# dariopagliaricci/Metal-PathTracer-arm64

Measured on AMD Instinct MI355X. Metric: Msamples/sec (whole node) at 1920×1080, depth 8; PFM RMSE vs Embree ref, higher is better.
Workload: dtype f32; 1 GPU; BASELINE configs[1]: Cornell box + one 70,688-triangle OBJ mesh, 1920x1080, depth 8, 256 spp, seed 1337; partition=8-row bands round-robin over 1 rank(s), RCCL gather of the HDR buffer

## Files before the change

### metal-pathtracer-arm64_amd/csrc/host/device_scene.h

```cpp
#pragma once

#include <hip/hip_runtime.h>

#include <cstdio>
#include <cstring>
#include <exception>
#include <functional>
#include <memory>
#include <string>
#include <vector>

#include "../kernels/device_types.h"
#include "../kernels/launch.h"
#include "env_importance_sampler.h"
#include "geometry_cache.h"
#include "ptr_abi.h"

namespace ptrhost {

struct HipError {
    std::string message;
};

#define HIP_CHECK(expr)                                                                                     \
// ... 88 lines not shown

}

struct PtrDeviceScene {
    int device = 0;
    DeviceBuffer<uint4> qnodes;
    DeviceBuffer<uint4> wnodes;
    DeviceBuffer<float4> nodes, tris, triNormals, spheres, materials, rects, rectLights, envRgba;
    DeviceBuffer<uint2> sphereInfo;
    DeviceBuffer<int32_t> lightIndexByRect;
    DeviceBuffer<float2> envCond, envMarg, cone;
    DeviceBuffer<float4> triUv, triTangent, texels, materialTex;
    DeviceBuffer<uint4> texInfo;
    DeviceBuffer<float> envPdf;
    DeviceBuffer<float4> envMips;
    uint32_t envMipLevels = 0;
    ptrk::SceneView view{};
    std::unique_ptr<ptrhost::DynamicScene> dynamic;
    uint64_t info[8] = {0};
    double uploadSeconds = 0.0;
    double timings[4] = {0.0, 0.0, 0.0, 0.0};
    uint64_t deviceTotalBytes = 0;
    bool hasRandomWalkMaterial = false;

    DeviceBuffer<float4> state, recBuf, itemAccum;
    DeviceBuffer<float2> hit;
    DeviceBuffer<uint32_t> flushItem, signature, tailList, tailWords;
    DeviceBuffer<uint32_t> connectList, connectCounts;
    DeviceBuffer<uint32_t> busyLists, busyCounts;
    uint64_t tailBelow = 512ull << 10;
    uint64_t poolSlots = 32ull << 20;
    uint32_t poolGroups = 0;
    bool connectOverlap = true;
    uint32_t maxPoolGroups() const { return poolGroups ? poolGroups : 4u; }
    uint32_t feederChunk = 256;
    std::vector<hipStream_t> groupStreams;
    std::vector<hipEvent_t> groupEvents;
    std::vector<hipStream_t> sideStreams;
    std::vector<hipEvent_t> sideEvents;
    int refillBelow = 40;
    uint32_t spillLevels = 0;
    uint32_t wideDepth = 0;
    DeviceBuffer<uint4> medium;
    DeviceBuffer<float> envLod;
    DeviceBuffer<uint32_t> scalars, pixelOfLocal, spill;
    DeviceBuffer<uint2> itemReserve;
    DeviceBuffer<uint32_t> itemHeads, zeros;
    DeviceBuffer<uint64_t> counters;
    DeviceBuffer<float> outBands;
    DeviceBuffer<float> covBands;
    DeviceBuffer<float4> covMean;
    ptrhost::AdaptiveStore adaptive;
    DeviceBuffer<float> adaptiveOut;
    DeviceBuffer<float4> rayBatch;
    DeviceBuffer<PtrHit> hitBatch;
    uint32_t* pinnedAlive = nullptr;
    uint32_t traceGrid = 0;
    uint32_t traceGridHalf = 0;
    uint32_t cachedW = 0, cachedH = 0, cachedPart = 0, cachedParts = 0, cachedLocalPixels = 0;

    ~PtrDeviceScene() {
        if (pinnedAlive) (void)hipHostFree(pinnedAlive);
        for (hipStream_t st : groupStreams) (void)hipStreamDestroy(st);
        for (hipEvent_t e : groupEvents) (void)hipEventDestroy(e);
        for (hipStream_t st : sideStreams) (void)hipStreamDestroy(st);
        for (hipEvent_t e : sideEvents) (void)hipEventDestroy(e);
// ... 73 lines not shown
```

### metal-pathtracer-arm64_amd/csrc/host/hip_backend.cpp

```cpp
#include <hip/hip_runtime.h>

#include <algorithm>
#include <chrono>
#include <cmath>
#include <cstdio>
#include <cstdlib>
#include <cstring>
#include <exception>
#include <memory>
#include <string>
#include <functional>
#include <vector>

#include "bvh_builder.h"
#include "device_scene.h"
#include "env_importance_sampler.h"
#include "geometry_cache.h"
#include "knobs.h"
#include "ptr_dynamic.h"
#include "scene_geometry.h"
#include "vecmath.h"

using namespace ptrk;
using namespace ptrhost;
// ... 257 lines not shown
        ds.texels.upload(reinterpret_cast<const float4*>(ps.texels.data()), ps.texels.size() / 4);
        ds.texInfo.upload(reinterpret_cast<const uint4*>(ps.texInfo.data()), ps.texInfo.size() / 4);
        ds.materialTex.upload(reinterpret_cast<const float4*>(ps.materialTex.data()), ps.materialTex.size() / 4);
        v.triUv = ds.triUv.ptr;
        v.triTangent = ds.triTangent.ptr;
        v.texels = ds.texels.ptr;
        v.texInfo = ds.texInfo.ptr;
        v.materialTex = ds.materialTex.ptr;
        v.textureCount = desc.textureCount;
    }

    if (ps.dynamic) uploadDynamicTables(ps, ds);

    ds.info[0] = bvh.nodeCount;
    ds.info[1] = bvh.leafCount;
    ds.info[2] = triCount;
    ds.info[3] = desc.sphereCount;
    ds.info[4] = bvh.maxDepth;
    ds.info[5] = bvh.maxLeafSize;
    ds.info[6] = static_cast<uint64_t>(bvh.sahCost * 1000.0);
    ds.info[7] = lightCount;

    hipDeviceProp_t prop;
    HIP_CHECK(hipGetDeviceProperties(&prop, ds.device));
    ds.deviceTotalBytes = prop.totalGlobalMem;
    const uint32_t cus = prop.multiProcessorCount > 0 ? static_cast<uint32_t>(prop.multiProcessorCount) : 256u;
    ds.traceGrid = cus * 8u;
    if (knobs.refillBelow > 0) ds.refillBelow = knobs.refillBelow;
    ds.traceGridHalf = cus * 4u;
    if (knobs.tailBelow >= 0) ds.tailBelow = static_cast<uint64_t>(knobs.tailBelow);
    if (knobs.poolSlots != 0) ds.poolSlots = knobs.poolSlots;
    if (knobs.poolGroups != 0) ds.poolGroups = knobs.poolGroups;
    ds.connectOverlap = knobs.connectOverlap != 0;
    const uint32_t wideLevels = ps.pg.wideCount > 0u ? ps.pg.wideDepth : 0u;
    const uint32_t stackNeed = std::min<uint32_t>(kTraversalStackDepth, std::max(3u * wideLevels, static_cast<uint32_t>(bvh.maxDepth)) + 4u);
    v.stackLimit = std::max(stackNeed, kLdsStackLevels);
    ds.wideDepth = wideLevels;
    ds.spillLevels = v.stackLimit - kLdsStackLevels;
    ds.spill.ensure(std::max<size_t>(spillWordsPerGroup(ds) * ds.maxPoolGroups() * 2u, 1u));
    ds.scalars.ensure(static_cast<size_t>(kScalarCount) * kMaxPoolGroups);
    ds.counters.ensure(kCounterSlots);
    ds.zeros.ensure(16);
    HIP_CHECK(hipMemset(ds.zeros.ptr, 0, 16 * sizeof(uint32_t)));
    HIP_CHECK(hipHostMalloc(reinterpret_cast<void**>(&ds.pinnedAlive), sizeof(uint32_t) * (kPinnedHeadsOffset + kItemHeads), hipHostMallocDefault));
    const double copySeconds = std::chrono::duration<double>(std::chrono::steady_clock::now() - t0).count();
    ds.uploadSeconds = ps.seconds + copySeconds;
    ds.timings[0] = ps.geometrySeconds;
    ds.timings[1] = ps.shadingSeconds;
    ds.timings[2] = copySeconds;
    ds.timings[3] = ps.geometryFromCache ? 1.0 : 0.0;
    if (knobs.verboseBuild) std::fprintf(stderr, "[upload] prepare %.2f s, copies to the device %.2f s\n", ps.seconds, copySeconds);
}

}

namespace {

int uploadTo(const char* who, const PtrSceneDesc* scene, const char* cachePath, int device, PtrDeviceScene** outScene, char* err, size_t cap,
             bool dynamic = false) {
    if (!scene || !outScene) return nullArgument(who, err, cap);
    if (ptr_device_count() <= device || device < 0) {
        setErr(err, cap, std::string(who) + ": no such HIP device (the HIP path has no CPU fallback)");
        return 2;
    }
    try {
        auto ds = std::make_unique<PtrDeviceScene>();
// ... 80 lines not shown
    rp.byWidth = makeDivU32(s.width);
    rp.height = s.height;
    rp.maxDepth = std::min(s.maxDepth, kFlagFieldMask);
    rp.shadowSlack = (s.debugShadowSlack > 0.0f && s.debugShadowSlack < 1.0f) ? s.debugShadowSlack : 0.0f;
    rp.seedBase = s.seed != 0 ? s.seed : 0x9e3779b9u;
    rp.spp = std::max(1u, spp);
    rp.sampleBase = 0u;
    rp.sppTotal = rp.spp;
    rp.passFlags = 3u;
    rp.enableRussianRoulette = s.enableRussianRoulette;
    rp.enableSpecularNee = s.enableSpecularNee;
    rp.enableMnee = s.enableMnee;
    rp.enableMneeSecondary = s.enableMneeSecondary;
    rp.backgroundMode = s.backgroundMode;
    std::memcpy(rp.backgroundColor, s.backgroundColor, sizeof(rp.backgroundColor));
    rp.envRotation = s.environmentRotation;
    rp.envIntensity = s.environmentIntensity;
    rp.clampFactor = std::max(s.fireflyClampFactor, 0.0f);
    rp.clampFloor = std::max(s.fireflyClampFloor, 0.0f);
    rp.throughputClamp = std::max(s.throughputClamp, 0.0f);
    rp.tailClampBase = std::max(s.specularTailClampBase, 0.0f);
    rp.tailClampRoughnessScale = std::max(s.specularTailClampRoughnessScale, 0.0f);
    rp.minSpecularPdf = std::max(s.minSpecularPdf, 1.0e-8f);
    rp.clampEnabled = s.fireflyClampEnabled ? 1.0f : 0.0f;
    rp.emissionScale = (s.emissionScale > 0.0f && std::isfinite(s.emissionScale)) ? s.emissionScale : 1.0f;
    rp.mediaMode = s.metalSemantics & (PTR_METAL_MEDIA | PTR_METAL_THIN | PTR_METAL_FACE_NORMAL | PTR_METAL_SPECULAR | PTR_METAL_SSS | PTR_METAL_PBR |
                                       PTR_METAL_CLAMPS | PTR_METAL_ENV_LOD | PTR_METAL_RAY_DIFF);
    rp.clampMaxContribution = std::max(s.fireflyClampMaxContribution, 0.0f);
    rp.minSpecularPdfRaw = s.minSpecularPdf;
    rp.sssMode = s.sssMode;
    rp.sssMaxSteps = std::max(s.sssMaxSteps, 1u);
}

LaunchConfig coldLaunchConfig(const PtrDeviceScene& ds) { return LaunchConfig{ds.traceGrid, ds.spill.ptr, ds.scalars.ptr + 1, ds.refillBelow}; }

void partitionPixels(uint32_t width, uint32_t height, uint32_t part, uint32_t parts, std::vector<uint32_t>& out) {
    out.clear();
    const uint32_t bands = (height + PTR_BAND_ROWS - 1u) / PTR_BAND_ROWS;
    for (uint32_t b = part; b < bands; b += parts) {
        const uint32_t y0 = b * PTR_BAND_ROWS, y1 = std::min(y0 + PTR_BAND_ROWS, height);
        for (uint32_t ty = y0; ty < y1; ty += 8u) {
            for (uint32_t tx = 0; tx < width; tx += 8u) {
                for (uint32_t y = ty; y < std::min(ty + 8u, y1); ++y) {
                    for (uint32_t x = tx; x < std::min(tx + 8u, width); ++x) out.push_back(y * width + x);
                }
            }
        }
    }
}

void addLaunchStats(PtrRenderStats& a, const PtrRenderStats& b) {
    a.traceKernelMs += b.traceKernelMs;
    a.shadeKernelMs += b.shadeKernelMs;
    a.shadowKernelMs += b.shadowKernelMs;
    a.tailKernelMs += b.tailKernelMs;
    a.traceLaunches += b.traceLaunches;
    a.samples += b.samples;
}

}

namespace {

uint64_t itemBudgetBytes(const PtrDeviceScene& ds) {
    return std::max<uint64_t>(64ull << 20, std::min<uint64_t>(16ull << 30, ds.deviceTotalBytes / 4u));
}

// ... 110 lines not shown
        ds.sideEvents.push_back(newEvent());
    }
}

std::vector<PoolGroup> makeGroups(PtrDeviceScene& ds, const RenderParams& rp, bool count, bool soloGroup, uint32_t slots, hipStream_t stream) {
    const uint32_t wantGroups = ds.poolGroups ? ds.poolGroups : (slots > (8u << 20) ? 2u : 4u);
    uint32_t groupCount = std::min<uint32_t>(soloGroup ? 1u : wantGroups, std::max<uint32_t>(1u, slots >> 20));
    const uint32_t groupSlots = ((slots + groupCount - 1u) / groupCount + 255u) & ~255u;
    groupCount = (slots + groupSlots - 1u) / groupSlots;
    const bool overlap = ds.connectOverlap && !soloGroup && groupCount <= 2u;
    ensureGroupStreams(ds, groupCount, overlap);
    const size_t spillWords = spillWordsPerGroup(ds);
    const uint32_t connectRegion = ((groupSlots + 63u) / 64u + kConnectQueues - 1u) / kConnectQueues * 64u;
    const size_t connectListWords = static_cast<size_t>(connectRegion) * kConnectQueues;
    if (slots >= (1u << kConnectMaskShift)) throw HipError{"path-slot pool too large for the connect lists"};
    ds.connectList.ensure(connectListWords * groupCount);
    ds.connectCounts.ensure(kConnectCountWords * 2u * kMaxPoolGroups);
    ds.busyLists.ensure(connectListWords * 2u * groupCount);
    ds.busyCounts.ensure(kConnectCountWords * 3u * kMaxPoolGroups);
    std::vector<PoolGroup> groups(groupCount);
    for (uint32_t g = 0; g < groupCount; ++g) {
        PoolGroup& gr = groups[g];
        const uint32_t first = g * groupSlots;
        gr.pool = slotRange(ds, rp, count, slots, first, std::min(groupSlots, slots - first), gr.env);
        gr.pool.connectList = ds.connectList.ptr + connectListWords * g;
        gr.pool.connectRegion = connectRegion;
        gr.listWords = connectListWords;
        gr.connectCounts = ds.connectCounts.ptr + kConnectCountWords * 2u * g;
        gr.busyLists = ds.busyLists.ptr + connectListWords * 2u * g;
        gr.busyCounts = ds.busyCounts.ptr + kConnectCountWords * 3u * g;
        gr.scalars = ds.scalars.ptr + static_cast<size_t>(g) * kScalarCount;
        const bool sideBySide = groupCount > 1 && gr.pool.slots >= kHalfGridGroupSlots;
        gr.cfg = LaunchConfig{sideBySide ? ds.traceGridHalf : ds.traceGrid, ds.spill.ptr + g * spillWords, gr.scalars + 1, ds.refillBelow};
        gr.stream = g == 0 ? stream : ds.groupStreams[g - 1];
        gr.feederChunk = ds.feederChunk;
        if (overlap) {
            gr.side = ds.sideStreams[g];
            gr.shadeDone = ds.sideEvents[2 * g];
            gr.connectDone = ds.sideEvents[2 * g + 1];
            gr.sideSpill = ds.spill.ptr + (ds.maxPoolGroups() + g) * spillWords;
        }
    }
    return groups;
}

uint64_t itemRangeStart(const RenderParams& rp, uint32_t k) {
    return std::min<uint64_t>(static_cast<uint64_t>(rp.itemHeadFirst) + static_cast<uint64_t>(k) * rp.itemsPerHead, rp.itemCount);
}

constexpr uint64_t kPollEvery = 4;
constexpr uint64_t kPollDry = 2;

struct PollResult {
    bool allDone, runTail, queueDry;
    uint64_t nextCheck;
};

PollResult poll(PtrDeviceScene& ds, std::vector<PoolGroup>& groups, const RenderParams& rp, uint32_t slots, uint64_t iterations, bool queueDry,
                bool tracePolls) {
    HIP_CHECK(hipGetLastError());
    const uint32_t ring = static_cast<uint32_t>((iterations - 1u) % kAliveRing);
    bool headsCopied = false;
    for (uint32_t g = 0; g < groups.size(); ++g) {
        PoolGroup& gr = groups[g];
        if (gr.done) continue;
        if (queueDry) {
// ... 527 lines not shown
```

### metal-pathtracer-arm64_amd/csrc/host/knobs.cpp

```cpp
#include "knobs.h"

#include <algorithm>
#include <cstdlib>
#include <cstring>

namespace ptr {

namespace {

long long numberOr(const char* name, long long fallback) {
    const char* e = std::getenv(name);
    if (!e || !*e) return fallback;
    char* end = nullptr;
    const long long v = std::strtoll(e, &end, 10);
    return end == e ? fallback : v;
}

bool hasTopic(const char* list, const char* topic) {
    if (!list) return false;
    const size_t n = std::strlen(topic);
    for (const char* p = list; *p;) {
        const char* q = std::strchr(p, ',');
        const size_t len = q ? static_cast<size_t>(q - p) : std::strlen(p);
        if ((len == n && std::strncmp(p, topic, n) == 0) || (len == 3 && std::strncmp(p, "all", 3) == 0)) return true;
        p += len + (q ? 1 : 0);
    }
    return false;
}

}

Knobs readKnobs() {
    Knobs k;
    k.poolSlots = static_cast<uint64_t>(std::min<long long>(std::max<long long>(numberOr("PTR_POOL_SLOTS", 0), 0), 64ll << 20));
    if (k.poolSlots != 0 && k.poolSlots < 1024) k.poolSlots = 1024;
    k.poolGroups = static_cast<uint32_t>(std::min<long long>(std::max<long long>(numberOr("PTR_POOL_GROUPS", 0), 0), 8));
    k.connectOverlap = static_cast<int>(numberOr("PTR_CONNECT_OVERLAP", -1));
    k.wideNodes = static_cast<int>(numberOr("PTR_WIDE_NODES", -1));
    k.quantizedNodes = static_cast<int>(numberOr("PTR_QUANTIZED_NODES", -1));
    k.tailBelow = numberOr("PTR_TAIL_BELOW", -1);
    k.maxItems = static_cast<uint64_t>(std::max<long long>(numberOr("PTR_MAX_ITEMS", 0), 0));
    if (k.maxItems != 0 && k.maxItems < 1024) k.maxItems = 1024;
    k.refillBelow = static_cast<int>(std::min<long long>(std::max<long long>(numberOr("PTR_REFILL_BELOW", 0), 0), 64));
    k.buildThreads = static_cast<uint32_t>(std::min<long long>(std::max<long long>(numberOr("PTR_BUILD_THREADS", 0), 0), 256));
    k.noOversize = numberOr("PTR_NO_OVERSIZE", 0) != 0;
    k.denoiseTiled = static_cast<int>(numberOr("PTR_DENOISE_TILED", -1));
    const char* verbose = std::getenv("PTR_VERBOSE");
    k.verboseBuild = hasTopic(verbose, "build");
    k.verbosePolls = hasTopic(verbose, "polls");
    k.verboseLaunches = hasTopic(verbose, "launches");
    k.verboseSteps = hasTopic(verbose, "steps");
    return k;
}

}
```

### metal-pathtracer-arm64_amd/csrc/host/knobs.h

```cpp
#pragma once

#include <cstdint>

namespace ptr {

struct Knobs {
    uint64_t poolSlots = 0;
    uint32_t poolGroups = 0;
    int connectOverlap = -1;
    int wideNodes = -1;
    int quantizedNodes = -1;
    int64_t tailBelow = -1;
    uint64_t maxItems = 0;
    int refillBelow = 0;
    uint32_t buildThreads = 0;
    bool noOversize = false;
    int denoiseTiled = -1;
    bool verboseBuild = false, verbosePolls = false, verboseLaunches = false, verboseSteps = false;
};

Knobs readKnobs();

}
```

### metal-pathtracer-arm64_amd/csrc/kernels/device_types.h

```cpp
#pragma once

#include <cstdint>
#include <hip/hip_runtime.h>

#include "bvh_layout.h"

namespace ptrk {

struct SceneView {
    const float4* nodes;
    const uint4* qnodes;
    float gridOrigin[3];
    float gridCell[3];
    float gridInvCell[3];
    uint32_t useQuantized;
    const float4* tris;
    const float4* triNormals;
    const float4* spheres;
    const uint2* sphereInfo;
    const float4* materials;
    const float4* rects;
    const float4* rectLights;
    const int32_t* lightIndexByRect;
    const float4* envRgba;
// ... 92 lines not shown
    uint32_t sssMode;
    uint32_t sssMaxSteps;
    uint32_t itemHeadFirst;
    uint32_t itemsPerHead;
    uint32_t enableRussianRoulette, enableSpecularNee, enableMnee, enableMneeSecondary;
    uint32_t backgroundMode;
    float backgroundColor[3];
    float envRotation, envIntensity;
    float clampFactor, clampFloor, throughputClamp, tailClampBase, tailClampRoughnessScale, minSpecularPdf, clampEnabled;
    float emissionScale;
    float clampMaxContribution, minSpecularPdfRaw;
    float shadowSlack;
};

struct EnvLodView {
    const float4* mips;
    float* slotLod;
    uint32_t levels;
    uint32_t pad;
};

struct ShadowRecordView {
    float4* org;
    float4* dir;
    float4* a;
    float4* b;
};

constexpr uint32_t kItemHeads = 64u;
constexpr uint32_t kItemHeadStride = 64u;
constexpr uint32_t kItemHeadWords = kItemHeads * kItemHeadStride + 1u;

constexpr uint32_t kRecSlots = 5u;

struct PathPool {
    float4* ray0;
    float4* ray1;
    float2* hit;
    float4* thr;
    float4* accum;
    uint32_t* flushItem;
    uint4* medium;
    float2* cone;
    uint32_t* signature;
    float4* itemAccum;
    uint32_t* nextItem;
    ShadowRecordView rec[kRecSlots];
    uint2* itemReserve;
    const uint32_t* pixelOfLocal;
    const float4* zero;
    uint64_t* counters;
    uint32_t slots;
    uint32_t recStride;
    uint32_t* connectList;
    uint32_t* connectCount;
    uint32_t* connectClear;
    uint32_t connectRegion;
    const uint32_t* busyIn;
    const uint32_t* busyCountIn;
    uint32_t* busyOut;
    uint32_t* busyCountOut;
    uint32_t* busyCountClear;
};
constexpr uint32_t kBusyAliveBit = 1u << 31;
constexpr uint32_t kConnectQueues = 64u;
constexpr uint32_t kConnectCountStride = 64u;
// ... 74 lines not shown
```

### metal-pathtracer-arm64_amd/csrc/kernels/launch.h

```cpp
#pragma once

#include <hip/hip_runtime.h>

#include "device_types.h"
#include "ptr_abi.h"

namespace ptrk {

struct LaunchConfig {
    uint32_t traceGrid;
    uint32_t* spill;
    uint32_t* workCounters;
    int refillBelow;
    uint32_t feederChunk = 256;
};

void launchGenerate(const RenderParams& rp, const PathPool& pool, hipStream_t stream);
int traversalNodeFormat(const SceneView& sc, bool count);
void launchExtend(const SceneView& sc, const PathPool& pool, const LaunchConfig& cfg, uint32_t* aliveOut, bool count, hipStream_t stream);
struct ShadeResets {
    uint32_t* extendHead;
    uint32_t* connectHead;
    uint32_t* nextAlive;
    uint32_t drained;
};
void launchShade(const RenderParams& rp, const SceneView& sc, const PathPool& pool, const ShadeResets& resets, const EnvLodView& env, bool count,
                 hipStream_t stream);
uint32_t shadeKernelSet(const RenderParams& rp, const SceneView& sc, bool count);
void launchConnect(const RenderParams& rp, const SceneView& sc, const PathPool& pool, const LaunchConfig& cfg, bool count,
                   hipStream_t stream);
void launchTail(const RenderParams& rp, const SceneView& sc, const PathPool& pool, const EnvLodView& env, const LaunchConfig& cfg, uint32_t* dList,
                uint32_t* dListCount, uint32_t* dListHead, bool count, hipStream_t stream);
void launchResolve(const RenderParams& rp, const PathPool& pool, uint32_t partCount, float* dOut, hipStream_t stream);
void launchResolveCov(const RenderParams& rp, const PathPool& pool, uint32_t partCount, float4* dMean, float* dCov, hipStream_t stream);

void launchTraceRays(const SceneView& sc, const float4* dRays, uint64_t n, bool anyHit, PtrHit* dOut, const LaunchConfig& cfg,
                     uint64_t* dCounters, hipStream_t stream);

void launchAovs(const RenderParams& rp, const SceneView& sc, uint32_t sample, float4* dAlbedo, float4* dNormal, const LaunchConfig& cfg,
                hipStream_t stream);

void launchDebugEvalBsdf(const float4* dMaterial, const RenderParams& rp, const float* dIn, uint64_t n, float* dOut,
                         hipStream_t stream);
void launchDebugSampleBsdf(const float4* dMaterial, const RenderParams& rp, const float* dIn, const uint32_t* dFront,
                           const uint32_t* dRng, uint64_t n, float* dOut, uint32_t* dRngOut, hipStream_t stream);
void launchDebugSampleLobes(const float4* dMaterial, const RenderParams& rp, const float* dIn, const uint32_t* dFront, const uint32_t* dRng,
                            uint64_t n, float* dOut, float* dSample, uint32_t* dRngOut, hipStream_t stream);
// ... 20 lines not shown
```

### metal-pathtracer-arm64_amd/csrc/kernels/wavefront.hip

```cpp
#include <hip/hip_runtime.h>

#include <algorithm>

#include "bsdf.h"
#include "device_types.h"
#include "launch.h"
#include <type_traits>
#include "traverse.h"
#include "texture.h"
#include "vec.h"

namespace ptrk {

namespace {

constexpr float kEps = 1.0e-4f;
constexpr float kSpecNeePdfFloor = 1.0e-4f;
constexpr float kSpecNeeInvPdfClamp = 1.0e4f;
constexpr float kMisMin = 1.0e-4f;
constexpr float kMisMax = 0.9999f;
#ifndef PTR_SHADE_BLOCK
#define PTR_SHADE_BLOCK 128
#endif
constexpr uint32_t kShadeBlock = PTR_SHADE_BLOCK;
// ... 1422 lines not shown
                        const bool dirValid = finite3(bs.dir);
                        const bool mneeEligible = rp.enableMnee && bs.isDelta && dirValid && type == 2u && nextSpecDepth == 1u;
                        const bool specNeeEligible = rp.enableSpecularNee && bs.isDelta && dirValid && !mneeEligible;

                        if (specNeeEligible || mneeEligible) {
                            const f3 sdir = normalize(bs.dir);
                            const f3 sorg = offsetOrigin(of, sdir);
                            if (envSampling) {
                                const SpecularLightWeight w = specularLightWeight(envPdfOf(sc, sdir, rp.envRotation), bs.pdf);
                                const f3 envColor = envLookup(sc, sdir, rp.envRotation, rp.envIntensity);
                                const f3 contrib = (bs.weight * envColor) * (w.mis * w.invPdf);
                                if (finite3(contrib)) {
                                    const f3 clamped = clampFirefly(thr, contrib, cc);
                                    if (clamped.x > 0.0f || clamped.y > 0.0f || clamped.z > 0.0f) {
                                        storeRecord(pool, slot, 2u, 0u, sorg, INFINITY, sdir, clamped, 0.0f, mk3(0.0f));
                                        want[2] = true;
                                    }
                                }
                            }
                            if (sc.rectLightCount > 0u && sc.settleRectLights) {
                                if (COUNT) counts.settled += 1u;
                                float tl;
                                uint32_t li = 0u, half = 0u;
                                if (nearestRectLight(sc, sorg, sdir, tl, li, half)) {
                                    uint32_t ignore;
                                    const Surface ls = rectLightSurface(sc, sorg, sdir, tl, li, half, ignore);
                                    const f3 c = rectContributionAt(rp, sc, cc, ls, sorg, bs.weight, bs.pdf, thr);
                                    if (c.x != 0.0f || c.y != 0.0f || c.z != 0.0f) {
                                        storeRecord(pool, slot, 3u, 3u, sorg, tl, sdir, c, 0.0f, mk3(__uint_as_float(ignore), 0.0f, 0.0f));
                                        want[3] = true;
                                    }
                                }
                            } else if (sc.rectLightCount > 0u) {
                                storeRecord(pool, slot, 3u, 1u, sorg, INFINITY, sdir, bs.weight, bs.pdf, thr);
                                want[3] = true;
                            }
                        }
                        if (mneeEligible && rp.enableMneeSecondary) {
                            const f3 sdir = normalize(bs.dir);
                            storeRecord(pool, slot, 4u, 2u, offsetOrigin(of, sdir), __uint_as_float(rng), sdir, bs.weight, bs.pdf, thr);
                            want[4] = true;
                        }

                        thr *= bs.weight;
                        thr = clampThroughput(thr, cc);
                        const float maxComp = smax(smax(thr.x, thr.y), thr.z);
                        if (!finite3(thr) || maxComp <= 0.0f) {
                            endPath = true;
                        } else {
                            lastPdf = bs.pdf > 0.0f ? bs.pdf : lastPdf;
                            lastDelta = bs.isDelta;
                            if (envLodOn && bs.lobe == 1 && !bs.isDelta && env.levels > 1u) {
                                envLodNext = envLodFromRoughness(bs.lobeRoughness, static_cast<float>(env.levels - 1u));
                            }
                            nextO = (SSS && bs.hasExit) ? sssExitOrigin(bs.exitPoint, n, bs.dir) : offsetOrigin(of, bs.dir);
                            nextD = bs.dir;
                            if (TEX && pool.cone) {
                                if (!haveCone) cone = pool.cone[slot];
                                haveCone = true;
                                cone.x = smax(cone.x + cone.y * smax(hitv.x, 0.0f), 1.0e-7f);
                                float inc = 0.0f;
                                if (!bs.isDelta) {
                                    const bool pbr = cc.metalPbr && type == 7u;
                                    const int lobe = pbr ? bs.lobe : ((type == 0u || type == 5u) ? 0 : 1);
                                    const float r = clampf(pbr ? bs.lobeRoughness : mat.roughness01(), 0.0f, 1.0f);
                                    inc = lobe == 0 ? 0.55f : (lobe == 1 ? 0.03f + (0.45f - 0.03f) * r : 0.10f + (0.60f - 0.10f) * r);
                                }
// ... 202 lines not shown
    f3 result = mk3(0.0f);
    if (COUNT) ++raysClosest;
    const TraceHit h = traverse<false, COUNT>(sc, org, dir, kEps, INFINITY, stack, cntClosest);
    if (h.prim == kHitMiss || sc.materialCount == 0u) return result;
    const Surface cs = reconstruct(sc, org, dir, h.t, h.prim);
    f3 tmpE;
    float tmpP;
    if (sc.rectLightCount > 0u && rectLightHit(sc, cs, org, rp.emissionScale, tmpE, tmpP)) return result;
    const Mat cm{sc.materials + static_cast<size_t>(min(cs.material, sc.materialCount - 1u)) * kMaterialVec4};
    if (!materialIsDelta(cm)) return result;
    f3 cn = cs.normal;
    if (dot(cn, cn) <= 0.0f) cn = mk3(0.0f, 1.0f, 0.0f);
    cn = normalize(cn);
    const f3 cin = normalize(dir);
    const BsdfSampleResult s2 = sampleBsdf(cm, cs.position, cn, -cin, cin, cs.frontFace, rngCopy, cc);
    if (!(s2.pdf > 0.0f && s2.isDelta && dot(s2.dir, s2.dir) > 0.0f && finite3(s2.weight))) return result;
    const f3 d2 = normalize(s2.dir);
    const f3 o2 = offsetOrigin(cs, d2);
    const f3 w2 = weight * s2.weight;
    const float pdf2 = bsdfPdf * s2.pdf;
    if (sc.envSampling) {
        if (COUNT) ++raysAny;
        result += alongEnv<COUNT>(rp, sc, cc, o2, d2, w2, pdf2, thr, stack, cntAny);
    }
    if (sc.rectLightCount > 0u) {
        if (COUNT) ++raysClosest;
        result += alongRect<COUNT>(rp, sc, cc, o2, d2, w2, pdf2, thr, stack, cntClosest);
    }
    return result;
}

}

template <bool COUNT, int NODES>
__global__ void __launch_bounds__(kTraceBlock) PTR_EXTEND_ATTR k_connect(RenderParams rp, SceneView sc, PathPool pool, uint32_t* spill, uint32_t spillStride,
                                                          uint32_t* workCounter, int kRefillBelow, uint32_t feederChunk) {
    __shared__ uint32_t ldsStack[kLdsStackLevels * kTraceBlock];
    LaneStack stack = laneStack(ldsStack, spill, spillStride, sc);
    TraceCounters cnt{0u, 0u}, cntClosest{0u, 0u};
    uint32_t rays = 0u, raysClosest = 0u, early = 0u;
    const ClampCfg cc = clampCfg(rp);

    SceneMem mem = sceneMem(sc);
    SubLists lists;
    lists.init(pool.connectCount, pool.connectRegion);
    WaveFeeder feeder;
    feeder.init(workCounter, lists.total, shortListChunk(lists.total, (gridDim.x * blockDim.x) >> 6));
    Trav t;
    t.cur = 0u;
    bool active = false;
    uint32_t mySlot = 0u, bits = 0u;
    float4* const recBase = pool.rec[0].org;
    const uint32_t slots = pool.recStride;
    uint32_t myRecAt = 0u;
    while (true) {
        const int nActive = __popcll(__ballot(active));
        const bool idleBits = __ballot(!active && bits != 0u) != 0ull;
        if (nActive < kRefillBelow && (idleBits || !feeder.exhausted)) {
            if (!feeder.exhausted) {
                const uint32_t idx = feeder.take(!active && bits == 0u);
                const uint32_t at = lists.position(idx != WaveFeeder::kNone ? idx : 0u, pool.connectRegion);
                if (idx != WaveFeeder::kNone) {
                    const uint32_t entry = pool.connectList[at];
                    mySlot = entry & ((1u << kConnectMaskShift) - 1u);
                    bits = entry >> kConnectMaskShift;
                }
            }
            if (!active && bits != 0u) {
                const uint32_t rec = static_cast<uint32_t>(__ffs(static_cast<int>(bits))) - 1u;
                bits &= bits - 1u;
                myRecAt = rec * 4u * slots + mySlot;
                const float4 o4 = recBase[myRecAt], d4 = recBase[myRecAt + slots];
                const uint32_t kind = __float_as_uint(d4.w);
                if (kind != 2u) {
                    const bool any = kind != 1u;
                    if (COUNT) { if (any) ++rays; else ++raysClosest; }
                    active = travBegin<NODES>(sc, t, mk3(o4), mk3(d4), kEps, any ? o4.w : INFINITY, any, stack);
                    if (kind == 3u) t.hit.prim = __float_as_uint(recBase[myRecAt + 3u * slots].x);
                    if (!active && kind == 1u) recBase[myRecAt + 2u * slots] = make_float4(0.0f, 0.0f, 0.0f, 0.0f);
                }
            }
            continue;
        }
        if (nActive == 0) break;
        {
            TraceCounters step{0u, 0u};
            const bool more = travVote<COUNT, NODES>(sc, mem, t, active, stack, step);
            if (COUNT) {
                TraceCounters& dst = t.anyHit ? cnt : cntClosest;
                dst.nodes += step.nodes;
                dst.prims += step.prims;
            }
            if (!more) {
                active = false;
                float4* const a = recBase + myRecAt + 2u * slots;
                if (t.anyHit) {
                    if (COUNT) early += anyHitFound(t.hit.prim) ? 1u : 0u;
                    if (anyHitFound(t.hit.prim)) *a = make_float4(0.0f, 0.0f, 0.0f, 0.0f);
                } else {
                    const float4 a4 = *a;
                    const f3 c = rectContribution(rp, sc, cc, t.org, t.dir, t.hit, mk3(a4), a4.w, mk3(recBase[myRecAt + 3u * slots]));
                    *a = mk4(c, 0.0f);
                }
            }
        }
    }
    addTraceCounters<COUNT>(pool.counters, rays, cnt, raysClosest, cntClosest);
    if (COUNT) addCounter(pool.counters, kCntShadowEarlyExit, early);
}

template <bool COUNT>
__global__ void __launch_bounds__(kTraceBlock) k_connect_chain(RenderParams rp, SceneView sc, PathPool pool, uint32_t* spill, uint32_t spillStride) {
    __shared__ uint32_t ldsStack[kLdsStackLevels * kTraceBlock];
    const uint32_t gtid = blockIdx.x * kTraceBlock + threadIdx.x;
    LaneStack stack = laneStack(ldsStack, spill, spillStride, sc);
    TraceCounters cnt{0u, 0u}, cntClosest{0u, 0u};
    uint32_t rays = 0u, raysClosest = 0u;
    const ClampCfg cc = clampCfg(rp);
    for (uint32_t slot = gtid; slot < pool.slots; slot += gridDim.x * kTraceBlock) {
        if (!((__float_as_uint(pool.ray1[slot].w) >> kFlagPendingShift) & (1u << 4))) continue;
        const ShadowRecordView& r = pool.rec[4];
        const float4 d4 = r.dir[slot];
        if (__float_as_uint(d4.w) != 2u) continue;
        const float4 o4 = r.org[slot], a4 = r.a[slot];
        const f3 c = mneeChain<COUNT>(rp, sc, cc, mk3(o4), mk3(d4), __float_as_uint(o4.w), mk3(a4), a4.w, mk3(r.b[slot]), stack, cnt,
                                      cntClosest, rays, raysClosest);
        r.a[slot] = mk4(c, 0.0f);
    }
    addTraceCounters<COUNT>(pool.counters, rays, cnt, raysClosest, cntClosest);
}

__global__ void __launch_bounds__(256) k_tail_collect(PathPool pool, uint32_t* list, uint32_t* listCount) {
    __shared__ uint32_t found[4][64];
    const uint32_t wave = threadIdx.x >> 6, lane = laneId();
    const uint32_t wavesTotal = gridDim.x * 4u;
    const uint32_t waveId = blockIdx.x * 4u + wave;
    const uint32_t perWave = ((pool.slots + wavesTotal - 1u) / wavesTotal + 63u) & ~63u;
    const uint32_t begin = waveId * perWave, end = min(begin + perWave, pool.slots);
    uint32_t have = 0u;
    auto flush = [&]() {
        uint32_t base = 0u;
// ... 554 lines not shown
    const uint32_t needs = sc.materialTypes | ((sc.envWidth > 0u || sc.envSampling) ? kFeatureEnvironment : 0u) |
                           ((rp.mediaMode & (PTR_METAL_MEDIA | PTR_METAL_FACE_NORMAL)) ? kFeatureMedia : 0u);
    for (uint32_t set : {kDiffuseMaterials, kBasicMaterials, kMetalMaterials, kCarPaintMaterials, kPbrMaterials}) {
        if ((needs & ~set) == 0u) {
            v.set = set;
            break;
        }
    }
    return v;
}

uint32_t shadeKernelSet(const RenderParams& rp, const SceneView& sc, bool count) { return shadeVariant(rp, sc, count).set; }

void launchShade(const RenderParams& rp, const SceneView& sc, const PathPool& pool, const ShadeResets& resets, const EnvLodView& env, bool count,
                 hipStream_t stream) {
    const ShadeVariant v = shadeVariant(rp, sc, count);
    const bool listed = pool.busyIn != nullptr;
    const uint32_t grid = ceilDiv(pool.slots, kShadeBlock);
    auto launch = [&](auto kernel) { hipLaunchKernelGGL(kernel, dim3(grid), dim3(kShadeBlock), 0, stream, rp, sc, pool, resets, env); };
    withBools([&](auto countTag, auto listedTag) {
        constexpr bool C = decltype(countTag)::value, L = decltype(listedTag)::value;
        if (v.tex) launch(k_shade<C, true, true, L>);
        else if (v.sss) launch(k_shade<C, true, false, L>);
        else if (C) launch(k_shade<C, false, false, L>);
        else if (v.set == kDiffuseMaterials) launch(k_shade<false, false, false, L, kDiffuseMaterials>);
        else if (v.set == kBasicMaterials) launch(k_shade<false, false, false, L, kBasicMaterials>);
        else if (v.set == kMetalMaterials) launch(k_shade<false, false, false, L, kMetalMaterials>);
        else if (v.set == kCarPaintMaterials) launch(k_shade<false, false, false, L, kCarPaintMaterials>);
        else if (v.set == kPbrMaterials) launch(k_shade<false, false, false, L, kPbrMaterials>);
        else launch(k_shade<C, false, false, L>);
    }, count, listed);
}

void launchConnect(const RenderParams& rp, const SceneView& sc, const PathPool& pool, const LaunchConfig& cfgIn, bool count, hipStream_t stream) {
    const TraceLaunch t = traceLaunch(cfgIn);
    withNodeFormat(sc, count, [&](auto countTag, auto nodesTag) {
        hipLaunchKernelGGL((k_connect<decltype(countTag)::value, decltype(nodesTag)::value>), dim3(t.grid), dim3(kTraceBlock), 0, stream, rp, sc, pool,
                           t.cfg.spill, t.stride, t.cfg.workCounters + 1, t.cfg.refillBelow, t.cfg.feederChunk);
    });
    if (rp.enableMnee && rp.enableMneeSecondary) {
        withBools([&](auto countTag) {
            hipLaunchKernelGGL(k_connect_chain<decltype(countTag)::value>, dim3(t.grid), dim3(kTraceBlock), 0, stream, rp, sc, pool, t.cfg.spill, t.stride);
        }, count);
    }
}

void launchTail(const RenderParams& rp, const SceneView& sc, const PathPool& pool, const EnvLodView& env, const LaunchConfig& cfgIn, uint32_t* dList,
                uint32_t* dListCount, uint32_t* dListHead, bool count, hipStream_t stream) {
    const TraceLaunch t = traceLaunch(cfgIn);
    const uint32_t collectGrid = std::max(1u, std::min(t.grid, ceilDiv(pool.slots, 256u * 16u)));
    hipLaunchKernelGGL(k_tail_collect, dim3(collectGrid), dim3(256), 0, stream, pool, dList, dListCount);
    const ShadeVariant v = shadeVariant(rp, sc, count);
    withBools([&](auto countTag, auto sssTag, auto texTag) {
        constexpr bool C = decltype(countTag)::value, S = decltype(sssTag)::value, T = decltype(texTag)::value;
        hipLaunchKernelGGL((k_tail_run<C, S, S && T>), dim3(t.grid), dim3(kTraceBlock), 0, stream, rp, sc, pool, dList, dListCount, dListHead,
                           t.cfg.spill, t.stride, env);
    }, count, v.sss, v.tex);
}

void launchResolve(const RenderParams& rp, const PathPool& pool, uint32_t partCount, float* dOut, hipStream_t stream) {
    hipLaunchKernelGGL(k_flush, dim3(ceilDiv(pool.slots, 256)), dim3(256), 0, stream, rp, pool);
    hipLaunchKernelGGL(k_resolve, dim3(ceilDiv(rp.localPixels, 256)), dim3(256), 0, stream, rp, pool, partCount, dOut);
}

void launchTraceRays(const SceneView& sc, const float4* dRays, uint64_t n, bool anyHit, PtrHit* dOut, const LaunchConfig& cfgIn,
                     uint64_t* dCounters, hipStream_t stream) {
    const TraceLaunch t = traceLaunch(cfgIn, n);
    withBools([&](auto anyTag) {
        hipLaunchKernelGGL(k_trace_rays<decltype(anyTag)::value>, dim3(t.grid), dim3(kTraceBlock), 0, stream, sc, dRays, n, dOut, t.cfg.spill, t.stride,
                           dCounters);
    }, anyHit);
}
// ... 78 lines not shown
```

Measured before the change: 2526 Msamples/s.

## Split rect-light contribution out of connect traversal into a settle kernel

The connect kernel no longer takes RenderParams or evaluates rect-light contributions inline. It is templated on whether closest-hit records are traced, and for closest hits it only stores the hit distance and primitive. A new k_connect_settle kernel then computes rectContribution for those records. This is meant to slim the traversal kernel (fewer registers, simpler code, and a variant that skips closest records entirely when they are not needed), at the cost of an extra launch and an extra round trip through memory for the records.

```diff
diff --git a/metal-pathtracer-arm64_amd/csrc/host/device_scene.h b/metal-pathtracer-arm64_amd/csrc/host/device_scene.h
--- a/metal-pathtracer-arm64_amd/csrc/host/device_scene.h
+++ b/metal-pathtracer-arm64_amd/csrc/host/device_scene.h
@@ -144,6 +144,7 @@
     uint64_t poolSlots = 32ull << 20;
     uint32_t poolGroups = 0;
     bool connectOverlap = true;
+    bool connectAllKinds = false;
     uint32_t maxPoolGroups() const { return poolGroups ? poolGroups : 4u; }
     uint32_t feederChunk = 256;
     std::vector<hipStream_t> groupStreams;
diff --git a/metal-pathtracer-arm64_amd/csrc/host/hip_backend.cpp b/metal-pathtracer-arm64_amd/csrc/host/hip_backend.cpp
--- a/metal-pathtracer-arm64_amd/csrc/host/hip_backend.cpp
+++ b/metal-pathtracer-arm64_amd/csrc/host/hip_backend.cpp
@@ -313,6 +313,7 @@
     if (knobs.poolSlots != 0) ds.poolSlots = knobs.poolSlots;
     if (knobs.poolGroups != 0) ds.poolGroups = knobs.poolGroups;
     ds.connectOverlap = knobs.connectOverlap != 0;
+    ds.connectAllKinds = knobs.connectAllKinds;
     const uint32_t wideLevels = ps.pg.wideCount > 0u ? ps.pg.wideDepth : 0u;
     const uint32_t stackNeed = std::min<uint32_t>(kTraversalStackDepth, std::max(3u * wideLevels, static_cast<uint32_t>(bvh.maxDepth)) + 4u);
     v.stackLimit = std::max(stackNeed, kLdsStackLevels);
@@ -459,7 +460,11 @@
     rp.sssMaxSteps = std::max(s.sssMaxSteps, 1u);
 }
 
-LaunchConfig coldLaunchConfig(const PtrDeviceScene& ds) { return LaunchConfig{ds.traceGrid, ds.spill.ptr, ds.scalars.ptr + 1, ds.refillBelow}; }
+LaunchConfig coldLaunchConfig(const PtrDeviceScene& ds) {
+    LaunchConfig cfg{ds.traceGrid, ds.spill.ptr, ds.scalars.ptr + 1, ds.refillBelow};
+    cfg.connectAllKinds = ds.connectAllKinds;
+    return cfg;
+}
 
 void partitionPixels(uint32_t width, uint32_t height, uint32_t part, uint32_t parts, std::vector<uint32_t>& out) {
     out.clear();
@@ -636,6 +641,7 @@
         gr.scalars = ds.scalars.ptr + static_cast<size_t>(g) * kScalarCount;
         const bool sideBySide = groupCount > 1 && gr.pool.slots >= kHalfGridGroupSlots;
         gr.cfg = LaunchConfig{sideBySide ? ds.traceGridHalf : ds.traceGrid, ds.spill.ptr + g * spillWords, gr.scalars + 1, ds.refillBelow};
+        gr.cfg.connectAllKinds = ds.connectAllKinds;
         gr.stream = g == 0 ? stream : ds.groupStreams[g - 1];
         gr.feederChunk = ds.feederChunk;
         if (overlap) {
diff --git a/metal-pathtracer-arm64_amd/csrc/host/knobs.cpp b/metal-pathtracer-arm64_amd/csrc/host/knobs.cpp
--- a/metal-pathtracer-arm64_amd/csrc/host/knobs.cpp
+++ b/metal-pathtracer-arm64_amd/csrc/host/knobs.cpp
@@ -36,6 +36,7 @@
     if (k.poolSlots != 0 && k.poolSlots < 1024) k.poolSlots = 1024;
     k.poolGroups = static_cast<uint32_t>(std::min<long long>(std::max<long long>(numberOr("PTR_POOL_GROUPS", 0), 0), 8));
     k.connectOverlap = static_cast<int>(numberOr("PTR_CONNECT_OVERLAP", -1));
+    k.connectAllKinds = numberOr("PTR_CONNECT_ALL_KINDS", 0) != 0;
     k.wideNodes = static_cast<int>(numberOr("PTR_WIDE_NODES", -1));
     k.quantizedNodes = static_cast<int>(numberOr("PTR_QUANTIZED_NODES", -1));
     k.tailBelow = numberOr("PTR_TAIL_BELOW", -1);
diff --git a/metal-pathtracer-arm64_amd/csrc/host/knobs.h b/metal-pathtracer-arm64_amd/csrc/host/knobs.h
--- a/metal-pathtracer-arm64_amd/csrc/host/knobs.h
+++ b/metal-pathtracer-arm64_amd/csrc/host/knobs.h
@@ -8,6 +8,7 @@
     uint64_t poolSlots = 0;
     uint32_t poolGroups = 0;
     int connectOverlap = -1;
+    bool connectAllKinds = false;
     int wideNodes = -1;
     int quantizedNodes = -1;
     int64_t tailBelow = -1;
diff --git a/metal-pathtracer-arm64_amd/csrc/kernels/device_types.h b/metal-pathtracer-arm64_amd/csrc/kernels/device_types.h
--- a/metal-pathtracer-arm64_amd/csrc/kernels/device_types.h
+++ b/metal-pathtracer-arm64_amd/csrc/kernels/device_types.h
@@ -148,6 +148,7 @@
 constexpr uint32_t kItemHeadWords = kItemHeads * kItemHeadStride + 1u;
 
 constexpr uint32_t kRecSlots = 5u;
+constexpr uint32_t kClosestRecord = 3u;
 
 struct PathPool {
     float4* ray0;
diff --git a/metal-pathtracer-arm64_amd/csrc/kernels/launch.h b/metal-pathtracer-arm64_amd/csrc/kernels/launch.h
--- a/metal-pathtracer-arm64_amd/csrc/kernels/launch.h
+++ b/metal-pathtracer-arm64_amd/csrc/kernels/launch.h
@@ -13,6 +13,7 @@
     uint32_t* workCounters;
     int refillBelow;
     uint32_t feederChunk = 256;
+    bool connectAllKinds = false;
 };
 
 void launchGenerate(const RenderParams& rp, const PathPool& pool, hipStream_t stream);
diff --git a/metal-pathtracer-arm64_amd/csrc/kernels/wavefront.hip b/metal-pathtracer-arm64_amd/csrc/kernels/wavefront.hip
--- a/metal-pathtracer-arm64_amd/csrc/kernels/wavefront.hip
+++ b/metal-pathtracer-arm64_amd/csrc/kernels/wavefront.hip
@@ -1478,7 +1478,7 @@
                                     }
                                 }
                             } else if (sc.rectLightCount > 0u) {
-                                storeRecord(pool, slot, 3u, 1u, sorg, INFINITY, sdir, bs.weight, bs.pdf, thr);
+                                storeRecord(pool, slot, kClosestRecord, 1u, sorg, INFINITY, sdir, bs.weight, bs.pdf, thr);
                                 want[3] = true;
                             }
                         }
@@ -1747,14 +1747,13 @@
 
 }
 
-template <bool COUNT, int NODES>
-__global__ void __launch_bounds__(kTraceBlock) PTR_EXTEND_ATTR k_connect(RenderParams rp, SceneView sc, PathPool pool, uint32_t* spill, uint32_t spillStride,
+template <bool COUNT, int NODES, bool CLOSEST>
+__global__ void __launch_bounds__(kTraceBlock) PTR_EXTEND_ATTR k_connect(SceneView sc, PathPool pool, uint32_t* spill, uint32_t spillStride,
                                                           uint32_t* workCounter, int kRefillBelow, uint32_t feederChunk) {
     __shared__ uint32_t ldsStack[kLdsStackLevels * kTraceBlock];
     LaneStack stack = laneStack(ldsStack, spill, spillStride, sc);
     TraceCounters cnt{0u, 0u}, cntClosest{0u, 0u};
     uint32_t rays = 0u, raysClosest = 0u, early = 0u;
-    const ClampCfg cc = clampCfg(rp);
 
     SceneMem mem = sceneMem(sc);
     SubLists lists;
@@ -1764,36 +1763,35 @@
     Trav t;
     t.cur = 0u;
     bool active = false;
-    uint32_t mySlot = 0u, bits = 0u;
+    uint32_t mine = 0u;
+    constexpr uint32_t kSlotMask = (1u << kConnectMaskShift) - 1u;
     float4* const recBase = pool.rec[0].org;
     const uint32_t slots = pool.recStride;
-    uint32_t myRecAt = 0u;
+    auto recordAt = [&]() {
+        return (static_cast<uint32_t>(__ffs(static_cast<int>(mine >> kConnectMaskShift))) - 1u) * 4u * slots + (mine & kSlotMask);
+    };
+    auto recordDone = [&]() { mine &= (((mine >> kConnectMaskShift) - 1u) << kConnectMaskShift) | kSlotMask; };
     while (true) {
         const int nActive = __popcll(__ballot(active));
-        const bool idleBits = __ballot(!active && bits != 0u) != 0ull;
+        const bool idleBits = __ballot(!active && mine > kSlotMask) != 0ull;
         if (nActive < kRefillBelow && (idleBits || !feeder.exhausted)) {
             if (!feeder.exhausted) {
-                const uint32_t idx = feeder.take(!active && bits == 0u);
+                const uint32_t idx = feeder.take(!active && mine <= kSlotMask);
                 const uint32_t at = lists.position(idx != WaveFeeder::kNone ? idx : 0u, pool.connectRegion);
-                if (idx != WaveFeeder::kNone) {
-                    const uint32_t entry = pool.connectList[at];
-                    mySlot = entry & ((1u << kConnectMaskShift) - 1u);
-                    bits = entry >> kConnectMaskShift;
-                }
+                if (idx != WaveFeeder::kNone) mine = pool.connectList[at];
             }
-            if (!active && bits != 0u) {
-                const uint32_t rec = static_cast<uint32_t>(__ffs(static_cast<int>(bits))) - 1u;
-                bits &= bits - 1u;
-                myRecAt = rec * 4u * slots + mySlot;
+            if (!active && mine > kSlotMask) {
+                const uint32_t myRecAt = recordAt();
                 const float4 o4 = recBase[myRecAt], d4 = recBase[myRecAt + slots];
                 const uint32_t kind = __float_as_uint(d4.w);
-                if (kind != 2u) {
-                    const bool any = kind != 1u;
+                if (kind != 2u && (CLOSEST || kind != 1u)) {
+                    const bool any = !CLOSEST || kind != 1u;
                     if (COUNT) { if (any) ++rays; else ++raysClosest; }
                     active = travBegin<NODES>(sc, t, mk3(o4), mk3(d4), kEps, any ? o4.w : INFINITY, any, stack);
                     if (kind == 3u) t.hit.prim = __float_as_uint(recBase[myRecAt + 3u * slots].x);
-                    if (!active && kind == 1u) recBase[myRecAt + 2u * slots] = make_float4(0.0f, 0.0f, 0.0f, 0.0f);
+                    if (CLOSEST && !active && kind == 1u) recBase[myRecAt + 3u * slots].w = __uint_as_float(kHitMiss);
                 }
+                if (!active) recordDone();
             }
             continue;
         }
@@ -1802,26 +1800,50 @@
             TraceCounters step{0u, 0u};
             const bool more = travVote<COUNT, NODES>(sc, mem, t, active, stack, step);
             if (COUNT) {
-                TraceCounters& dst = t.anyHit ? cnt : cntClosest;
+                TraceCounters& dst = (!CLOSEST || t.anyHit) ? cnt : cntClosest;
                 dst.nodes += step.nodes;
                 dst.prims += step.prims;
             }
             if (!more) {
                 active = false;
-                float4* const a = recBase + myRecAt + 2u * slots;
-                if (t.anyHit) {
+                const uint32_t myRecAt = recordAt();
+                recordDone();
+                if (!CLOSEST || t.anyHit) {
                     if (COUNT) early += anyHitFound(t.hit.prim) ? 1u : 0u;
-                    if (anyHitFound(t.hit.prim)) *a = make_float4(0.0f, 0.0f, 0.0f, 0.0f);
+                    if (anyHitFound(t.hit.prim)) recBase[myRecAt + 2u * slots] = make_float4(0.0f, 0.0f, 0.0f, 0.0f);
                 } else {
-                    const float4 a4 = *a;
-                    const f3 c = rectContribution(rp, sc, cc, t.org, t.dir, t.hit, mk3(a4), a4.w, mk3(recBase[myRecAt + 3u * slots]));
-                    *a = mk4(c, 0.0f);
+                    recBase[myRecAt].w = t.hit.t;
+                    recBase[myRecAt + 3u * slots].w = __uint_as_float(t.hit.prim);
                 }
             }
         }
     }
     addTraceCounters<COUNT>(pool.counters, rays, cnt, raysClosest, cntClosest);
     if (COUNT) addCounter(pool.counters, kCntShadowEarlyExit, early);
+}
+
+__global__ void __launch_bounds__(kTraceBlock) k_connect_settle(RenderParams rp, SceneView sc, PathPool pool) {
+    const ClampCfg cc = clampCfg(rp);
+    SubLists lists;
+    lists.init(pool.connectCount, pool.connectRegion);
+    float4* const recBase = pool.rec[0].org;
+    const uint32_t slots = pool.recStride;
+    for (uint32_t first = (blockIdx.x * kTraceBlock + threadIdx.x) & ~63u; first < lists.total; first += gridDim.x * kTraceBlock) {
+        const uint32_t idx = first + laneId();
+        const bool mine = idx < lists.total;
+        const uint32_t at = lists.position(mine ? idx : 0u, pool.connectRegion);
+        const uint32_t entry = mine ? pool.connectList[at] : 0u;
+        if ((entry >> kConnectMaskShift) & (1u << kClosestRecord)) {
+            const uint32_t recAt = kClosestRecord * 4u * slots + (entry & ((1u << kConnectMaskShift) - 1u));
+            const float4 d4 = recBase[recAt + slots];
+            if (__float_as_uint(d4.w) == 1u) {
+                const float4 o4 = recBase[recAt], a4 = recBase[recAt + 2u * slots], b4 = recBase[recAt + 3u * slots];
+                const TraceHit h{o4.w, __float_as_uint(b4.w)};
+                const f3 c = rectContribution(rp, sc, cc, mk3(o4), mk3(d4), h, mk3(a4), a4.w, mk3(b4));
+                recBase[recAt + 2u * slots] = mk4(c, 0.0f);
+            }
+        }
+    }
 }
 
 template <bool COUNT>
@@ -2442,12 +2464,21 @@
     }, count, listed);
 }
 
+static bool connectTracesClosest(const RenderParams& rp, const SceneView& sc, bool count) {
+    return sc.rectLightCount > 0u && !sc.settleRectLights && (shadeRecords(shadeVariant(rp, sc, count).set) & (1u << kClosestRecord)) != 0u;
+}
+
 void launchConnect(const RenderParams& rp, const SceneView& sc, const PathPool& pool, const LaunchConfig& cfgIn, bool count, hipStream_t stream) {
     const TraceLaunch t = traceLaunch(cfgIn);
+    const bool closest = cfgIn.connectAllKinds || connectTracesClosest(rp, sc, count);
     withNodeFormat(sc, count, [&](auto countTag, auto nodesTag) {
-        hipLaunchKernelGGL((k_connect<decltype(countTag)::value, decltype(nodesTag)::value>), dim3(t.grid), dim3(kTraceBlock), 0, stream, rp, sc, pool,
-                           t.cfg.spill, t.stride, t.cfg.workCounters + 1, t.cfg.refillBelow, t.cfg.feederChunk);
+        withBools([&](auto closestTag) {
+            hipLaunchKernelGGL((k_connect<decltype(countTag)::value, decltype(nodesTag)::value, decltype(closestTag)::value>), dim3(t.grid),
+                               dim3(kTraceBlock), 0, stream, sc, pool, t.cfg.spill, t.stride, t.cfg.workCounters + 1, t.cfg.refillBelow,
+                               t.cfg.feederChunk);
+        }, closest);
     });
+    if (closest) hipLaunchKernelGGL(k_connect_settle, dim3(traceLaunch(cfgIn, pool.slots).grid), dim3(kTraceBlock), 0, stream, rp, sc, pool);
     if (rp.enableMnee && rp.enableMneeSecondary) {
         withBools([&](auto countTag) {
             hipLaunchKernelGGL(k_connect_chain<decltype(countTag)::value>, dim3(t.grid), dim3(kTraceBlock), 0, stream, rp, sc, pool, t.cfg.spill, t.stride);
```

Result: no change. 2542 Msamples/s, median of 6 (+0.7%).
